# zixinz990/quaternion-mpc

Measured on AMD Instinct MI355X. Metric: MPC QP solves/sec (Go1, 12 forces, N=10), higher is better.
Workload: dtype f64

## Files before the change

quaternion-mpc_amd/csrc/qmpc_device.h:

```cpp
#pragma once

#include <hip/hip_runtime.h>
#include <stdint.h>

#include "../../include/qmpc.h"
#include "qmpc_params_dev.h"

namespace qmpc {

constexpr int kWave = 64;

template <class... Tables>
hipError_t set_max_lds(const Tables&... tables) {
  hipError_t e = hipSuccess;
  auto one = [&e](const auto& table) {
    for (auto k : table)
      if (e == hipSuccess) e = hipFuncSetAttribute(reinterpret_cast<const void*>(k), hipFuncAttributeMaxDynamicSharedMemorySize, 160 * 1024);
  };
  (one(tables), ...);
  return e;
}

constexpr int LD = 16;
constexpr int MAT = 12 * LD;
// ... 55 lines not shown
  L.total = (o + 1) & ~1;
  return L;
}

enum {
  C_FOOT = 0,
  C_GB = 12,
  C_WD0 = 15,
  C_CR = 18,
  C_CON = 36,
  C_X0 = 40,
};

#define QSYNC() __syncthreads()

__device__ __forceinline__ void mtm_load(const double* X, const double* Y, int lane, d4& acc) {
  const double x0 = X[lane], x1 = X[64 + lane], x2 = X[128 + lane];
  const double y0 = Y[lane], y1 = Y[64 + lane], y2 = Y[128 + lane];
  acc = __builtin_amdgcn_mfma_f64_16x16x4f64(x0, y0, acc, 0, 0, 0);
  acc = __builtin_amdgcn_mfma_f64_16x16x4f64(x1, y1, acc, 0, 0, 0);
  acc = __builtin_amdgcn_mfma_f64_16x16x4f64(x2, y2, acc, 0, 0, 0);
}
__device__ __forceinline__ d4 mtm3(const double X[3], const double Y[3], d4 acc) {
  acc = __builtin_amdgcn_mfma_f64_16x16x4f64(X[0], Y[0], acc, 0, 0, 0);
  acc = __builtin_amdgcn_mfma_f64_16x16x4f64(X[1], Y[1], acc, 0, 0, 0);
  acc = __builtin_amdgcn_mfma_f64_16x16x4f64(X[2], Y[2], acc, 0, 0, 0);
  return acc;
}
__device__ __forceinline__ void mtm(double* C, const double* X, const double* Y, int lane) {
  d4 acc = {0.0, 0.0, 0.0, 0.0};
  mtm_load(X, Y, lane, acc);
  C[lane] = acc[0];
  C[64 + lane] = acc[1];
  C[128 + lane] = acc[2];
}

typedef unsigned u2v __attribute__((ext_vector_type(2)));

template <int CTRL>
__device__ __forceinline__ double dpp_mov(double x) {
  if constexpr (CTRL >= 0x150 && CTRL <= 0x15F) {
    return __builtin_amdgcn_update_dpp(0.0, x, CTRL, 0xF, 0xF, true);
  } else {
    int lo = __double2loint(x), hi = __double2hiint(x);
    lo = __builtin_amdgcn_update_dpp(0, lo, CTRL, 0xF, 0xF, true);
    hi = __builtin_amdgcn_update_dpp(0, hi, CTRL, 0xF, 0xF, true);
    return __hiloint2double(hi, lo);
  }
}
__device__ __forceinline__ void swap16(double x, double& even, double& odd) {
  const u2v lo = __builtin_amdgcn_permlane16_swap((unsigned)__double2loint(x), (unsigned)__double2loint(x), false, false);
  const u2v hi = __builtin_amdgcn_permlane16_swap((unsigned)__double2hiint(x), (unsigned)__double2hiint(x), false, false);
  even = __hiloint2double((int)hi[0], (int)lo[0]);
  odd = __hiloint2double((int)hi[1], (int)lo[1]);
}
__device__ __forceinline__ void swap32(double x, double& lower, double& upper) {
  const u2v lo = __builtin_amdgcn_permlane32_swap((unsigned)__double2loint(x), (unsigned)__double2loint(x), false, false);
  const u2v hi = __builtin_amdgcn_permlane32_swap((unsigned)__double2hiint(x), (unsigned)__double2hiint(x), false, false);
  lower = __hiloint2double((int)hi[0], (int)lo[0]);
  upper = __hiloint2double((int)hi[1], (int)lo[1]);
}
template <int G>
__device__ __forceinline__ double rowgroup_bcast(double x) {
  double ev, od, lo, up;
  swap16(x, ev, od);
  swap32((G & 1) ? od : ev, lo, up);
  return (G & 2) ? up : lo;
}

struct OpMin { __device__ __forceinline__ double operator()(double a, double b) const { return fmin(a, b); } };
struct OpMax { __device__ __forceinline__ double operator()(double a, double b) const { return fmax(a, b); } };
struct OpSum { __device__ __forceinline__ double operator()(double a, double b) const { return a + b; } };
template <class Op>
__device__ __forceinline__ double wave_reduce(double v, Op op) {
  v = op(v, dpp_mov<0xB1>(v));
  v = op(v, dpp_mov<0x4E>(v));
  v = op(v, dpp_mov<0x141>(v));
  v = op(v, dpp_mov<0x140>(v));
  double a, b;
  swap16(v, a, b);
  v = op(a, b);
  swap32(v, a, b);
  return op(a, b);
}
__device__ __forceinline__ double wave_min(double v) { return wave_reduce(v, OpMin()); }
__device__ __forceinline__ double wave_max(double v) { return wave_reduce(v, OpMax()); }
__device__ __forceinline__ double wave_sum(double v) { return wave_reduce(v, OpSum()); }

__device__ __forceinline__ double fast_rcp(double x) {
  double r = __builtin_amdgcn_rcp(x);
  r = fma(fma(-x, r, 1.0), r, r);
  r = fma(fma(-x, r, 1.0), r, r);
  return r;
}

__device__ __forceinline__ double fast_rsqrt(double x) {
  double r = __builtin_amdgcn_rsq(x);
  r = r * fma(-0.5 * x * r, r, 1.5);
  r = r * fma(-0.5 * x * r, r, 1.5);
  return r;
}

template <int J>
__device__ __forceinline__ double row_bcast(double x) {
  return dpp_mov<0x150 + J>(x);
}
template <int J, int ROWS>
__device__ __forceinline__ double row_bcast_rows(double x, double keep) {
  return __builtin_amdgcn_update_dpp(keep, x, 0x150 + J, ROWS, 0xF, false);
}
__device__ __forceinline__ double read_lane(double x, int l) {
  const int lo = __builtin_amdgcn_readlane(__double2loint(x), l);
  const int hi = __builtin_amdgcn_readlane(__double2hiint(x), l);
  return __hiloint2double(hi, lo);
}

__device__ __forceinline__ void quat_G(const double* q, double G[12]) {
  const double s = q[0], x = q[1], y = q[2], z = q[3];
  G[0] = -x; G[1] = -y;  G[2] = -z;
  G[3] = s;  G[4] = -z;  G[5] = y;
  G[6] = z;  G[7] = s;   G[8] = -x;
  G[9] = -y; G[10] = x;  G[11] = s;
}
__device__ __forceinline__ void quat_Omega(const double* w, double O[16]) {
  const double x = w[0], y = w[1], z = w[2];
  O[0] = 0;  O[1] = -x; O[2] = -y;  O[3] = -z;
  O[4] = x;  O[5] = 0;  O[6] = z;   O[7] = -y;
  O[8] = y;  O[9] = -z; O[10] = 0;  O[11] = x;
  O[12] = z; O[13] = y; O[14] = -x; O[15] = 0;
}

template <int NL, bool LEAN>
struct ModelRegsT {
  double gb[3], wd0[3], rm[LEAN ? 3 * NL : 9 * NL];
  __device__ __forceinline__ void load(const double* cst, const double* bw0) {
    typedef Dim<NL> D;
#pragma unroll
    for (int i = 0; i < 3; ++i) { gb[i] = cst[D::C_GB + i]; wd0[i] = cst[D::C_WD0 + i]; }
    if (LEAN) {
#pragma unroll
      for (int i = 0; i < 3 * NL; ++i) rm[i] = cst[D::C_CON + i / 3] * cst[D::C_FOOT + i];
    } else {
#pragma unroll
      for (int i = 0; i < 9 * NL; ++i) rm[i] = bw0[i];
    }
  }
};

template <int NL, bool LEAN>
__device__ __forceinline__ void srbd_step(const DevParams& P, const ModelRegsT<NL, LEAN>& M, const double* x,
                                          const double* u, double* xn) {
  double F[3], vd[3], wd[3];
  {
    double f0[2] = {0, 0}, f1[2] = {0, 0}, f2[2] = {0, 0};
#pragma unroll
    for (int l = 0; l < NL; ++l) { f0[l & 1] += u[3 * l]; f1[l & 1] += u[3 * l + 1]; f2[l & 1] += u[3 * l + 2]; }
    F[0] = f0[0] + f0[1]; F[1] = f1[0] + f1[1]; F[2] = f2[0] + f2[1];
    if (LEAN) {
      double t0[2] = {0, 0}, t1[2] = {0, 0}, t2[2] = {0, 0};
#pragma unroll
      for (int l = 0; l < NL; ++l) {
        const double* r = &M.rm[3 * l];
        const double* f = &u[3 * l];
        t0[l & 1] += r[1] * f[2] - r[2] * f[1];
        t1[l & 1] += r[2] * f[0] - r[0] * f[2];
        t2[l & 1] += r[0] * f[1] - r[1] * f[0];
// ... 684 lines not shown
```

quaternion-mpc_amd/csrc/qmpc_wform.h:

```cpp
#pragma once

namespace qmpc {


struct LayoutW {
  int GK, WR, SLW;
};
constexpr int kGK = 27;
template <int NL = 4>
__host__ __device__ inline size_t wform_slice(int N, bool sl_global = false) {
  return ((size_t)N * (13 * 12 + 21 * NL + kGK + (sl_global ? 18 * NL : 0)) + 1 + 1) & ~(size_t)1;
}
template <int NL = 4>
__host__ __device__ inline Layout make_layout_w(int N, LayoutW* W, bool kd_global = false, bool sl_global = false, bool cv = false,
                                                bool full = false) {
  Layout L;
  int o = 0;
  auto take = [&](int n) { int r = o; o += n; return r; };
  constexpr int nu = 3 * NL, nc = 6 * NL, nl = NL;
  L.cst = take(NL == 4 ? 64 : 80);
  L.bw0 = take(3 * nu);
  L.refp = take(13);
  L.uref = take(nu);
  L.X = take((N + 1) * 13);
  L.U = take(N * nu);
  L.Xc = take((N + 1) * 13);
  L.dU = take(N * nu);
  const bool lean = ((NL == 8) && !full) || sl_global;
  if (sl_global) {
    L.S = 0; L.LAM = N * nc; L.RC = 2 * N * nc;
  } else {
    L.S = take(N * nc);
    L.LAM = take(N * nc);
  }
  L.DS = lean ? -1 : take(N * nc);
  L.DLAM = lean ? -1 : take(N * nc);
  if (!sl_global) L.RC = take(N * nc);
  L.AB = take(N * kAB);
  L.XT = take((N + 1) * kXT);
  if (kd_global) {
    L.KD = 0; L.ROT = N * 13 * 12; W->GK = N * (13 * 12 + 21 * nl);
    W->SLW = (N * (13 * 12 + 21 * nl + kGK) + 1 + 1) & ~1;
  } else {
    L.KD = take(N * 13 * 12);
    L.ROT = take(N * 21 * nl);
    W->GK = take(N * kGK + 1);
  }
  W->WR = take(N * 6);
  L.CV = cv ? take(N * 8) : -1;
  L.tile = sl_global ? L.X : L.S;
  L.total = (o + 1) & ~1;
  return L;
}
template <int NL = 4>
__device__ __forceinline__ int zeta_slot(int k, int i) { return 21 * NL * k + 21 * (i / 3) + 18 + (i % 3); }

constexpr int S6I_(int i, int j) { return i * 6 - i * (i - 1) / 2 + (j - i); }
__host__ __device__ constexpr int S6I(int i, int j) { return i <= j ? S6I_(i, j) : S6I_(j, i); }

enum { WM_QUAT = 0, WM_CONVEX = 1 };
__host__ __device__ constexpr int cvperm(int r) { return r < 3 ? r + 3 : (r < 6 ? r - 3 : (r < 9 ? r + 3 : r - 3)); }
__device__ __forceinline__ void cv_step_w(const DevParams& P, const double* x, const double w[6], double* xn) {
  double s0, c0, w00, w01, w11;
  sincos(x[2], &s0, &c0);
  ConvexModel::winv(P, c0, s0, w00, w01, w11);
  const double vd[3] = {w[0] * P.inv_mass, w[1] * P.inv_mass, w[2] * P.inv_mass - 9.81};
  const double wd0[3] = {w00 * w[3] + w01 * w[4], w01 * w[3] + w11 * w[4], P.Iinv[8] * w[5]};
  const double yawm = x[2] + P.hh * x[8];
  const double wm[3] = {x[6] + P.hh * wd0[0], x[7] + P.hh * wd0[1], x[8] + P.hh * wd0[2]};
  double sm_, cm_;
  sincos(yawm, &sm_, &cm_);
  ConvexModel::winv(P, cm_, sm_, w00, w01, w11);
  const double wdm[3] = {w00 * w[3] + w01 * w[4], w01 * w[3] + w11 * w[4], P.Iinv[8] * w[5]};
  xn[0] = x[0] + P.h * (cm_ * wm[0] + sm_ * wm[1]);
  xn[1] = x[1] + P.h * (-sm_ * wm[0] + cm_ * wm[1]);
  xn[2] = x[2] + P.h * wm[2];
#pragma unroll
  for (int a = 0; a < 3; ++a) {
    xn[3 + a] = x[3 + a] + P.h * (x[9 + a] + P.hh * vd[a]);
    xn[6 + a] = x[6 + a] + P.h * wdm[a];
    xn[9 + a] = x[9 + a] + P.h * vd[a];
  }
  xn[12] = 0.0;
}
__device__ __forceinline__ void cv_winv_mul(const double* W, const double t[3], double y[3]) {
  y[0] = W[0] * t[0] + W[1] * t[1];
  y[1] = W[1] * t[0] + W[2] * t[1];
  y[2] = W[3] * t[2];
}

template <bool AL = false, int NL = 4, int MD = WM_QUAT, bool LEAN = (NL == 8)>
__device__ inline void prepass_w(const DevParams& P, const Layout& L, double* sm, const double* sl,
                                 double* ROT, double* GK, double target, int lane, unsigned kapbits = 0) {
  typedef Dim<NL> D;
  constexpr int LSH = (NL == 8) ? 3 : 2;
  static_assert(NL == 4 || NL == 8, "contact points per knot: one lane quad or two");
  const int N = P.N;
  const double* cst = sm + L.cst;
  double cr[18];
#pragma unroll
  for (int i = 0; i < 18; ++i) cr[i] = cst[D::C_CR + i];
  for (int q0 = 0; q0 < NL * N; q0 += kWave) {
    const int q = q0 + lane;
    const bool live = q < NL * N;
    const int k = live ? (q >> LSH) : 0, l = q & (NL - 1);
    double* out = ROT + D::ROT * k + 21 * l;
    double acc[kGK];
#pragma unroll
    for (int i = 0; i < kGK; ++i) acc[i] = 0.0;
    const bool stance = live && cst[D::C_CON + l] != 0.0;
    if (live && !stance) {
      out[0] = 1; out[1] = 0; out[2] = 0; out[3] = 0; out[4] = 1; out[5] = 0; out[6] = 0; out[7] = 0; out[8] = 1;
      out[9] = 0; out[10] = 0; out[11] = 0; out[12] = 1; out[13] = 1; out[14] = 1; out[15] = 0; out[16] = 0; out[17] = 0;
    }
    if (stance) {
      const int lr = (NL == 4) ? l : (l & 3);
      const double R0 = P.R[3 * lr], R1 = P.R[3 * lr + 1], R2 = P.R[3 * lr + 2];
      double w[6], gi[6];
#pragma unroll
      for (int i = 0; i < 6; ++i) {
        const double lam = sl[L.LAM + D::NC * k + 6 * l + i];
        const double rc = sl[L.RC + D::NC * k + 6 * l + i];
        if (AL) {
          const double z = lam + target * rc;
          w[i] = (z > 0.0) ? target : 0.0;
          gi[i] = (z > 0.0) ? z : 0.0;
        } else {
          const double s = sl[L.S + D::NC * k + 6 * l + i];
          const double kap = LEAN ? (((kapbits >> (6 * (q0 >> 6) + i)) & 1u) ? 1.0 : 0.0) : sl[L.DS + D::NC * k + 6 * l + i];
          const double is = fast_rcp(s);
          w[i] = lam * is;
          gi[i] = (target + lam * rc) * is - kap * lam;
        }
      }
      int i1 = 0;
      double w1 = w[0];
#pragma unroll
      for (int i = 1; i < 6; ++i) if (w[i] > w1) { w1 = w[i]; i1 = i; }
      int i2 = -1;
      double w2 = -1.0;
#pragma unroll
      for (int i = 0; i < 6; ++i) {
        const bool skip = (i == i1) || ((i1 >= 4) && (i >= 4));
        if (!skip && w[i] > w2) { w2 = w[i]; i2 = i; }
      }
      double a1[3] = {0, 0, 0}, a2[3] = {0, 0, 0};
#pragma unroll
      for (int i = 0; i < 6; ++i)
#pragma unroll
        for (int a = 0; a < 3; ++a) {
          a1[a] = (i == i1) ? cr[3 * i + a] : a1[a];
          a2[a] = (i == i2) ? cr[3 * i + a] : a2[a];
        }
      const double in1 = fast_rsqrt(a1[0] * a1[0] + a1[1] * a1[1] + a1[2] * a1[2]);
      double q1[3], q2[3], q3[3];
#pragma unroll
      for (int a = 0; a < 3; ++a) q1[a] = a1[a] * in1;
#pragma unroll
      for (int pass = 0; pass < 2; ++pass) {
        const double dp = a2[0] * q1[0] + a2[1] * q1[1] + a2[2] * q1[2];
#pragma unroll
        for (int a = 0; a < 3; ++a) a2[a] -= dp * q1[a];
      }
      const double in2 = fast_rsqrt(a2[0] * a2[0] + a2[1] * a2[1] + a2[2] * a2[2]);
#pragma unroll
      for (int a = 0; a < 3; ++a) q2[a] = a2[a] * in2;
      q3[0] = q1[1] * q2[2] - q1[2] * q2[1];
      q3[1] = q1[2] * q2[0] - q1[0] * q2[2];
      q3[2] = q1[0] * q2[1] - q1[1] * q2[0];
      double T[9];
#pragma unroll
      for (int a = 0; a < 3; ++a) { T[3 * a] = q1[a]; T[3 * a + 1] = q2[a]; T[3 * a + 2] = q3[a]; }
      const double Rl[3] = {R0, R1, R2};
      const double* u = sm + L.U + D::NU * k + 3 * l;
      const double* ur = sm + L.uref + 3 * l;
      const double ru[3] = {R0 * (u[0] - ur[0]), R1 * (u[1] - ur[1]), R2 * (u[2] - ur[2])};
      double gq[3];
      double d00, d01, d02, d11, d12, d22;
      {
        double tr[9];
#pragma unroll
        for (int i = 0; i < 9; ++i) tr[i] = T[i] * Rl[i / 3];
        d00 = tr[0] * T[0] + tr[3] * T[3] + tr[6] * T[6];
        d01 = tr[0] * T[1] + tr[3] * T[4] + tr[6] * T[7];
        d02 = tr[0] * T[2] + tr[3] * T[5] + tr[6] * T[8];
        d11 = tr[1] * T[1] + tr[4] * T[4] + tr[7] * T[7];
        d12 = tr[1] * T[2] + tr[4] * T[5] + tr[7] * T[8];
        d22 = tr[2] * T[2] + tr[5] * T[5] + tr[8] * T[8];
      }
#pragma unroll
      for (int a = 0; a < 3; ++a) gq[a] = T[a] * ru[0] + T[3 + a] * ru[1] + T[6 + a] * ru[2];
#pragma unroll
      for (int i = 0; i < 6; ++i) {
        double at[3];
#pragma unroll
        for (int b = 0; b < 3; ++b) at[b] = T[b] * cr[3 * i] + T[3 + b] * cr[3 * i + 1] + T[6 + b] * cr[3 * i + 2];
#pragma unroll
        for (int a = 0; a < 3; ++a) gq[a] += gi[i] * at[a];
        const double w0 = w[i] * at[0], w1_ = w[i] * at[1];
        d00 += w0 * at[0]; d01 += w0 * at[1]; d02 += w0 * at[2];
        d11 += w1_ * at[1]; d12 += w1_ * at[2];
        d22 += w[i] * at[2] * at[2];
      }
      const double id0 = fast_rcp(d00);
      const double l10 = d01 * id0, l20 = d02 * id0;
      const double e11 = d11 - l10 * d01;
      const double id1 = fast_rcp(e11);
      const double e21 = d12 - l20 * d01;
      const double l21 = e21 * id1;
      const double e22 = d22 - l20 * d02 - l21 * e21;
      const double id2 = fast_rcp(e22);
#pragma unroll
      for (int i = 0; i < 9; ++i) out[i] = T[i];
      out[9] = l10; out[10] = l20; out[11] = l21; out[12] = id0; out[13] = id1; out[14] = id2;
      out[15] = gq[0]; out[16] = gq[1]; out[17] = gq[2];
      double V[18];
#pragma unroll
      for (int i = 0; i < 9; ++i) V[i] = T[i];
      {
        const double* bw = sm + L.bw0 + 3 * l;
#pragma unroll
        for (int a = 0; a < 3; ++a)
#pragma unroll
          for (int b = 0; b < 3; ++b)
            V[9 + 3 * a + b] = bw[D::NU * a] * T[b] + bw[D::NU * a + 1] * T[3 + b] + bw[D::NU * a + 2] * T[6 + b];
        if (MD == WM_CONVEX) {
          const double* Wk = sm + L.CV + 8 * k;
#pragma unroll
          for (int b = 0; b < 3; ++b) {
            const double t3[3] = {V[9 + b], V[12 + b], V[15 + b]};
            double y[3];
            cv_winv_mul(Wk, t3, y);
            V[9 + b] = y[0]; V[12 + b] = y[1]; V[15 + b] = y[2];
          }
        }
      }
      const double y0 = gq[0], y1 = gq[1] - l10 * y0, y2 = gq[2] - l20 * y0 - l21 * y1;
      const double z0 = id0 * y0, z1 = id1 * y1, z2 = id2 * y2;
      double v0[6], v1[6], v2[6];
#pragma unroll
      for (int i = 0; i < 6; ++i) {
        v0[i] = V[3 * i];
        v1[i] = V[3 * i + 1] - l10 * v0[i];
        v2[i] = V[3 * i + 2] - l20 * v0[i] - l21 * v1[i];
        acc[21 + i] = v0[i] * z0 + v1[i] * z1 + v2[i] * z2;
      }
#pragma unroll
      for (int i = 0; i < 6; ++i) {
        const double b0 = id0 * v0[i], b1 = id1 * v1[i], b2 = id2 * v2[i];
#pragma unroll
        for (int j = i; j < 6; ++j) acc[S6I(i, j)] = b0 * v0[j] + b1 * v1[j] + b2 * v2[j];
      }
    }
#pragma unroll
    for (int i = 0; i < kGK; ++i) {
      double v = acc[i];
      v += dpp_mov<0xB1>(v);
      v += dpp_mov<0x4E>(v);
      if (NL == 8) v += dpp_mov<0x141>(v);
      acc[i] = v;
    }
    if (live && l == 0) {
      double* gk = GK + kGK * k;
#pragma unroll
      for (int i = 0; i < kGK; ++i) gk[i] = acc[i];
    }
  }
  QSYNC();
}

template <bool PROF>
__device__ __forceinline__ void tick_dep(Prof<PROF>& prof, int ph, double& a, double& b) {
  if (PROF) {
    asm volatile("s_nop 0" : "+v"(a), "+v"(b));
    prof.tick(ph);
    asm volatile("s_nop 0" : "+v"(a), "+v"(b));
  }
}

template <bool PROF>
__device__ __forceinline__ void tick_dep1(Prof<PROF>& prof, int ph, double& a) {
  if (PROF) {
    asm volatile("s_nop 0" : "+v"(a));
    prof.tick(ph);
    asm volatile("s_nop 0" : "+v"(a));
  }
}

__device__ __forceinline__ d4 mtm2(const double X[2], const double Y[2], d4 acc) {
  acc = __builtin_amdgcn_mfma_f64_16x16x4f64(X[0], Y[0], acc, 0, 0, 0);
  acc = __builtin_amdgcn_mfma_f64_16x16x4f64(X[1], Y[1], acc, 0, 0, 0);
  return acc;
}
__device__ __forceinline__ d4 acc_rows(double a, double b) {
  d4 v;
  v[0] = a; v[1] = b;
  return v;
}
__device__ __forceinline__ d4 acc_rows(double a, double b, double c) {
  d4 v;
  v[0] = a; v[1] = b; v[2] = c;
  return v;
}
struct ColOps {
  double m1c, m2c, keep, hsel;
  __device__ __forceinline__ void init(const DevParams& P, int c) {
    const double m1 = P.h * (P.hh * (1.0 / P.mass)), m2 = P.h * (1.0 / P.mass);
    m1c = (c < 3) ? m1 : 0.0;
    m2c = (c < 3) ? m2 : ((c < 6) ? P.h : 0.0);
    keep = (c >= 3 && c < 6) ? 0.0 : 1.0;
    hsel = (c >= 6 && c < 9) ? P.h : 0.0;
  }
};
constexpr int kZeroSlots = 54;
template <int NL> __host__ __device__ constexpr int kZeroSlotsT() { return NL == 4 ? kZeroSlots : 70; }
struct BwPat {
  ColOps co;
  double Mc[3], Nc[2], qadd[3], sel[3];
  int ix_w, st_w, ix_a, st_a, ix_x[3], st_x[3], ix_g[2], st_g[2], kwo[2], xoffN[3];
  bool c12;
  template <int NL = 4, int MD = WM_QUAT>
  __device__ __forceinline__ void init(const DevParams& P, const Layout& L, int lane) {
    const int N = P.N;
    const int c = lane & 15, g = lane >> 4;
    co.init(P, c);
    const int zs = L.cst + kZeroSlotsT<NL>();
    const bool c35 = (c >= 3 && c < 6), c911 = (c >= 9 && c < 12);
    c12 = c == 12;
    const int abN = L.AB + kAB * (N - 1);
    ix_w = c35 ? abN + 18 + (c - 3) : zs;   st_w = c35 ? kAB : 0;
    ix_a = c35 ? abN + (c - 3) : (c911 ? abN + 9 + (c - 9) : zs);   st_a = (c35 || c911) ? kAB : 0;
    sel[0] = (g == 3) ? 1.0 : 0.0;
    sel[1] = (g == 0) ? 1.0 : 0.0;
    sel[2] = (g == 1) ? 1.0 : 0.0;
    const double m1 = P.h * (P.hh * (1.0 / P.mass)), m2 = P.h * (1.0 / P.mass);
#pragma unroll
    for (int e = 0; e < 3; ++e) {
      const int r = 4 * e + g;
      const bool phi = (r >= 3 && r < 6);
      double v = 0.0;
      if (c < 6) {
        if (r < 3) v = (r == c) ? m1 : 0.0;
        else if (r >= 6 && r < 9) v = (r - 6 == c) ? m2 : 0.0;
        else if (r >= 9) v = (r - 9 == c - 3) ? P.h : 0.0;
      }
      Mc[e] = v;
      if (MD == WM_CONVEX) qadd[e] = (c < 12 && r == c) ? P.Q[cvperm(r < 12 ? r : 0)] : 0.0;
      else qadd[e] = (c < 12 && r == c && !phi) ? P.Q[(r < 3) ? r : r + 1] : 0.0;
      const bool xv = (MD == WM_CONVEX) ? c12 : ((phi && c35) || c12);
      const int xo = c12 ? 9 + r : 3 * (r - 3) + (c - 3);
      xoffN[e] = xv ? xo : -1;
      ix_x[e] = xv ? L.XT + kXT * (N - 1) + xo : zs;
      st_x[e] = xv ? kXT : 0;
    }
#pragma unroll
    for (int e = 0; e < 2; ++e) {
      const int r = 4 * e + g;
      const bool phi = (r >= 3 && r < 6);
      Nc[e] = (r < 3 && c == r + 6) ? P.h : ((phi && r == c) ? -1.0 : 0.0);
      const bool gv = r < 6 && (c < 6 || c12);
      const int go = c12 ? 21 + r : S6I(r < 6 ? r : 0, c < 6 ? c : 0);
      ix_g[e] = gv ? kGK * (N - 1) + go : kGK * N;
      st_g[e] = gv ? kGK : 0;
      kwo[e] = (r < 6 && c < 13) ? 13 * r + c : -1;
    }
  }
};
__device__ __forceinline__ void fma_bcast345_x2(double r[2], const double x[2], const double sh[2], double cs, const double m[3]) {
  asm("v_fmac_f64 %0, %4, %5\n\t"
      "v_fmac_f64 %1, %4, %6\n\t"
      "v_fmac_f64_dpp %0, %2, %7 row_newbcast:3 row_mask:0xf bank_mask:0xf\n\t"
      "v_fmac_f64_dpp %1, %3, %7 row_newbcast:3 row_mask:0xf bank_mask:0xf\n\t"
      "v_fmac_f64_dpp %0, %2, %8 row_newbcast:4 row_mask:0xf bank_mask:0xf\n\t"
      "v_fmac_f64_dpp %1, %3, %8 row_newbcast:4 row_mask:0xf bank_mask:0xf\n\t"
      "v_fmac_f64_dpp %0, %2, %9 row_newbcast:5 row_mask:0xf bank_mask:0xf\n\t"
      "v_fmac_f64_dpp %1, %3, %9 row_newbcast:5 row_mask:0xf bank_mask:0xf"
      : "+v"(r[0]), "+v"(r[1])
      : "v"(x[0]), "v"(x[1]), "v"(cs), "v"(sh[0]), "v"(sh[1]), "v"(m[0]), "v"(m[1]), "v"(m[2]));
}
__device__ __forceinline__ void fma_bcast345_x3(double r[3], const double x[3], const double sh[3], double cs, const double m[3]) {
  asm("v_fmac_f64 %0, %6, %7\n\t"
      "v_fmac_f64 %1, %6, %8\n\t"
      "v_fmac_f64 %2, %6, %9\n\t"
      "v_fmac_f64_dpp %0, %3, %10 row_newbcast:3 row_mask:0xf bank_mask:0xf\n\t"
      "v_fmac_f64_dpp %1, %4, %10 row_newbcast:3 row_mask:0xf bank_mask:0xf\n\t"
      "v_fmac_f64_dpp %2, %5, %10 row_newbcast:3 row_mask:0xf bank_mask:0xf\n\t"
      "v_fmac_f64_dpp %0, %3, %11 row_newbcast:4 row_mask:0xf bank_mask:0xf\n\t"
      "v_fmac_f64_dpp %1, %4, %11 row_newbcast:4 row_mask:0xf bank_mask:0xf\n\t"
      "v_fmac_f64_dpp %2, %5, %11 row_newbcast:4 row_mask:0xf bank_mask:0xf\n\t"
      "v_fmac_f64_dpp %0, %3, %12 row_newbcast:5 row_mask:0xf bank_mask:0xf\n\t"
      "v_fmac_f64_dpp %1, %4, %12 row_newbcast:5 row_mask:0xf bank_mask:0xf\n\t"
      "v_fmac_f64_dpp %2, %5, %12 row_newbcast:5 row_mask:0xf bank_mask:0xf"
      : "+v"(r[0]), "+v"(r[1]), "+v"(r[2])
      : "v"(x[0]), "v"(x[1]), "v"(x[2]), "v"(cs), "v"(sh[0]), "v"(sh[1]), "v"(sh[2]), "v"(m[0]), "v"(m[1]), "v"(m[2]));
}
__device__ __forceinline__ void times_M(const double x[2], const ColOps& co, const double wt[3], double r[2]) {
  double sh[2];
#pragma unroll
// ... 644 lines not shown
    o[0] = du[0]; o[1] = du[1]; o[2] = du[2];
    bad = bad || !(isfinite(du[0]) && isfinite(du[1]) && isfinite(du[2]));
    stp = fmax(stp, fmax(fabs(du[0]), fmax(fabs(du[1]), fabs(du[2]))));
#pragma unroll
    for (int i = 0; i < 6; ++i) {
      const double jd = cr[3 * i] * du[0] + cr[3 * i + 1] * du[1] + cr[3 * i + 2] * du[2];
      double dsv = -(jd + rc[i]);
      double dlv = (target - (1.0 + kap[i]) * sv[i] * lv[i] - lv[i] * dsv) * fast_rcp(sv[i]);
      dsv = stance ? dsv : 0.0;
      dlv = stance ? dlv : 0.0;
      const bool up = (dsv < 0.0) && (pd == 0.0 || sv[i] * pd < pn * (-dsv));
      pn = up ? sv[i] : pn; pd = up ? -dsv : pd;
      const bool ud = (dlv < 0.0) && (dd == 0.0 || lv[i] * dd < dn * (-dlv));
      dn = ud ? lv[i] : dn; dd = ud ? -dlv : dd;
      if (!LEAN) {
        sl[L.DS + i0 + i] = dsv;
        sl[L.DLAM + i0 + i] = dlv;
      }
      bits |= (stance && kap[i] != 0.0) ? (1u << (6 * j + i)) : 0u;
    }
  }
  const double ap = (pd > 0.0) ? fmin(1.0, P.tau * pn * fast_rcp(pd)) : 1.0;
  const double ad = (dd > 0.0) ? fmin(1.0, P.tau * dn * fast_rcp(dd)) : 1.0;
  *alpha_p = wave_min(ap);
  *alpha_d = wave_min(ad);
  *full_step = wave_max(stp);
  kapbits = bits;
  QSYNC();
  return __any(bad ? 1 : 0);
}

template <int NL = 4, bool LEAN = (NL == 8)>
__device__ inline void apply_w(const DevParams& P, const Layout& L, double* sl, double ap, double ad, unsigned conmask,
                               int lane, unsigned& kapbits, double& sl_part, double& rc_part, const double* sm = nullptr,
                               double target = 0.0) {
  typedef Dim<NL> D;
  constexpr int LSH = (NL == 8) ? 3 : 2;
  const int N = P.N;
  sl_part = 0.0;
  rc_part = 0.0;
  const bool full = (ap >= 0.99) && (ad >= 0.99);
  const double rcs = (ap >= 1.0) ? 0.0 : (1.0 - ap);
  int j = 0;
  for (int q = lane; q < NL * N; q += kWave, ++j) {
    const int k = q >> LSH, l = q & (NL - 1);
    if (!(conmask & (1u << l))) continue;
    const int i0 = D::NC * k + 6 * l;
    double s0[6], l0[6], ds[6], dl[6], rc[6];
#pragma unroll
    for (int i = 0; i < 6; ++i) {
      s0[i] = sl[L.S + i0 + i]; l0[i] = sl[L.LAM + i0 + i]; rc[i] = sl[L.RC + i0 + i];
      if (!LEAN) { ds[i] = sl[L.DS + i0 + i]; dl[i] = sl[L.DLAM + i0 + i]; }
    }
    if (LEAN) {
      const double* cr = sm + L.cst + D::C_CR;
      const double* du = sm + L.dU + D::NU * k + 3 * l;
      const double du0 = du[0], du1 = du[1], du2 = du[2];
#pragma unroll
      for (int i = 0; i < 6; ++i) {
        const double kp = ((kapbits >> (6 * j + i)) & 1u) ? 1.0 : 0.0;
        const double jd = cr[3 * i] * du0 + cr[3 * i + 1] * du1 + cr[3 * i + 2] * du2;
        ds[i] = -(jd + rc[i]);
        dl[i] = (target - (1.0 + kp) * s0[i] * l0[i] - l0[i] * ds[i]) * fast_rcp(s0[i]);
      }
    }
    unsigned newbits = 0;
#pragma unroll
    for (int i = 0; i < 6; ++i) {
      const bool kap0 = (kapbits >> (6 * j + i)) & 1u;
      const double s1 = s0[i] + ap * ds[i];
      const double l1 = l0[i] + ad * dl[i];
      const double rc1 = (ap >= 1.0) ? 0.0 : rcs * rc[i];
      sl[L.S + i0 + i] = s1;
      sl[L.RC + i0 + i] = rc1;
      sl[L.LAM + i0 + i] = l1;
      sl_part += s1 * l1;
      rc_part = fmax(rc_part, fabs(rc1));
      const bool sig = full && (s1 < 0.6 * s0[i]) && (l1 < 0.6 * l0[i]) && (kap0 || ((s1 > 0.4 * s0[i]) && (l1 > 0.4 * l0[i])));
      if (LEAN) newbits |= sig ? (1u << (6 * j + i)) : 0u;
      else sl[L.DS + i0 + i] = sig ? 1.0 : 0.0;
    }
    if (LEAN) kapbits = (kapbits & ~(63u << (6 * j))) | newbits;
  }
}

__device__ __forceinline__ int trial_states_slot(const Layout& L, int g) {
  return g == 0 ? L.Xc + 13 : (g == 1 ? L.S : (g == 2 ? L.DLAM : L.XT));
}
template <int MD = WM_QUAT, int NL = 4>
__device__ inline double rollout_trials_w(const DevParams& P, const Layout& L, const LayoutW& LW, double* sm,
                                          const double* KD, double* ZG, double alpha_g, int lane) {
  typedef typename std::conditional<MD == WM_CONVEX, ConvexModel, typename std::conditional<NL == 8, Quat8Model, QuatModel>::type>::type TM;
  typedef Dim<NL> D;
  const int N = P.N;
  const double* cst = sm + L.cst;
  double gb[3], wd0[3];
#pragma unroll
  for (int a = 0; a < 3; ++a) { gb[a] = cst[D::C_GB + a]; wd0[a] = cst[D::C_WD0 + a]; }
  const int r = lane & 15, g = lane >> 4;
  const int row = (r < 12) ? r : 0, wi = (r < 6) ? r : 0;
  double* zg = ZG + 6 * N * g;
  double* xg = sm + trial_states_slot(L, g);
  double xc[13], xn[13];
#pragma unroll
  for (int i = 0; i < 13; ++i) xc[i] = cst[D::C_X0 + i];
  if (lane == 15)
#pragma unroll
    for (int i = 0; i < 13; ++i) sm[L.Xc + i] = xc[i];
  double Jx = TM::knot_cost(P, sm + L.refp, sm + L.uref, 0, xc, nullptr);
  auto knot = [&](int k, RollLoadsW& cur) {
    roll_load_w(L, LW, sm, KD, k, row, wi, cur);
    double dx[12], e[12];
    if (MD == WM_CONVEX) {
#pragma unroll
      for (int rr = 0; rr < 12; ++rr) dx[rr] = xc[cvperm(rr)] - cur.xo[cvperm(rr)];
    } else {
      QuatModel::state_diff(cur.xo, xc, dx);
    }
#pragma unroll
    for (int a = 0; a < 3; ++a) {
      e[a] = dx[a] + P.h * dx[6 + a];
      e[3 + a] = (cur.ab[3 * a] * dx[3] + cur.ab[3 * a + 1] * dx[4] + cur.ab[3 * a + 2] * dx[5]) +
                 (cur.ab[9 + 3 * a] * dx[9] + cur.ab[9 + 3 * a + 1] * dx[10] + cur.ab[9 + 3 * a + 2] * dx[11]);
      e[6 + a] = dx[6 + a];
      e[9 + a] = dx[9 + a];
    }
    const double* kd = cur.kd;
    const double p0 = alpha_g * kd[12] + kd[0] * e[0] + kd[1] * e[1] + kd[2] * e[2];
    const double p1 = kd[3] * e[3] + kd[4] * e[4] + kd[5] * e[5];
    const double p2 = kd[6] * e[6] + kd[7] * e[7] + kd[8] * e[8];
    const double p3 = kd[9] * e[9] + kd[10] * e[10] + kd[11] * e[11];
    const double s = (p0 + p1) + (p2 + p3);
    const double wn = (MD == WM_CONVEX) ? s : cur.wk + s;
    if (r >= 6 && r < 12) zg[6 * k + r - 6] = s;
    double w[6];
    w[0] = dpp_mov<0x150>(wn); w[1] = dpp_mov<0x151>(wn); w[2] = dpp_mov<0x152>(wn);
    w[3] = dpp_mov<0x153>(wn); w[4] = dpp_mov<0x154>(wn); w[5] = dpp_mov<0x155>(wn);
    if (MD == WM_CONVEX) {
      RollLoadsC rc;
      roll_load_c(L, LW, sm, k, rc);
      const double d3 = rc.iw[0] * w[3] + rc.iw[1] * w[4], d4 = rc.iw[1] * w[3] + rc.iw[2] * w[4], d5 = rc.iw[3] * w[5];
      w[0] += rc.wr[0]; w[1] += rc.wr[1]; w[2] += rc.wr[2];
      w[3] = rc.wr[3] + d3; w[4] = rc.wr[4] + d4; w[5] = rc.wr[5] + d5;
      cv_step_w(P, xc, w, xn);
    } else
    srbd_step_w(P, gb, wd0, xc, w, xn);
#pragma unroll
    for (int i = 0; i < 13; ++i) xc[i] = xn[i];
    if (r == 15)
#pragma unroll
      for (int i = 0; i < 13; ++i) xg[13 * k + i] = xn[i];
    Jx += TM::knot_cost(P, sm + L.refp, sm + L.uref, k + 1, xc, nullptr);
  };
  RollLoadsW ra;
  for (int k = 0; k < N; ++k) knot(k, ra);
  QSYNC();
  return Jx;
}

template <int MD = WM_QUAT, int NL = 4>
__device__ inline void trial_inputs_w(const DevParams& P, const Layout& L, const double* sm, const double* sl,
                                      const double* ROT, const double* ZG, const double* Rl, double alpha, double rho,
                                      int lane, double Ju[4], double mer[4], double vi[4]) {
  typedef Dim<NL> D;
  constexpr int LSH = (NL == 8) ? 3 : 2;
  const int N = P.N;
// ... 139 lines not shown
```

quaternion-mpc_amd/csrc/qmpc_wform_body.inc:

```
#ifndef QMPC_WNL
#define QMPC_WNL 4
#define QMPC_WNL_DEFAULTED 1
#endif
#ifndef QMPC_WMODEL
#define QMPC_WMODEL WM_QUAT
#define QMPC_WMODEL_DEFAULTED 1
#endif
  constexpr int WNL = QMPC_WNL;
  constexpr int WMT = QMPC_WMODEL;
  typedef typename std::conditional<WMT == WM_CONVEX, ConvexModel, QuatModelT<WNL>>::type WMD;
  typedef Dim<WNL> WD;
  constexpr int NU = WD::NU, NC = WD::NC;
  const int N = P.N;
  constexpr bool KDG = WVAR == 5 || WVAR == 6;
  constexpr bool SLG = WVAR == 6;
  constexpr bool LEAN = WNL == 8 || SLG;
  LayoutW LW;
  const Layout L = make_layout_w<WNL>(N, &LW, KDG, SLG, WMT == WM_CONVEX);
  double* wsb = KDG ? gws + (size_t)wslot * wform_slice<WNL>(N, SLG) : sm;
  double* KD = wsb + L.KD;
  double* ROT = wsb + L.ROT;
  double* GK = wsb + LW.GK;
  double* sl = SLG ? wsb + LW.SLW : sm;
  const void* in = reinterpret_cast<const double*>(in_) + (size_t)b * WD::REC;
  int status = QMPC_OK;
  Prof<PROF> prof;
  prof.start();
  setup_instance<WMD>(P, L, sm, in, lane, &status);
  if (status != QMPC_OK) {
    if (lane < NU) forces[NU * (size_t)b + lane] = 0.0;
    if (lane == 0 && info) {
      qmpc_info r = {status, 0, 0.0, 0.0, 0.0, 0.0};
      info[b] = r;
    }
    if (traj_u) for (int i = lane; i < N * NU; i += kWave) traj_u[(size_t)b * N * NU + i] = 0.0;
    if (traj_x) for (int i = lane; i < (N + 1) * WMD::NX; i += kWave) traj_x[(size_t)b * (N + 1) * WMD::NX + i] = 0.0;
    return;
  }
  unsigned conmask = 0;
  for (int l = 0; l < WMD::NL; ++l) conmask |= (sm[L.cst + WD::C_CON + l] != 0.0) ? (1u << l) : 0u;
  conmask = __builtin_amdgcn_readfirstlane(conmask);
  if (lane < 10) sm[L.cst + kZeroSlotsT<WNL>() + lane] = 0.0;
  if (lane == 0) GK[kGK * N] = 0.0;
  BwPat bp;
  if (!KDG) bp.init<WNL, WMT>(P, L, lane);
  if (resume) {
    for (int i = lane; i < N * NU; i += kWave) sm[L.U + i] = resume[8 + i];
  } else if (warm_t > 0) {
    if (lane < NU) {
      const bool stance = (conmask >> (lane / 3)) & 1u;
      for (int k = 0; k < N; ++k) {
        const double prev = sm[L.U + ((k + 1 < N) ? k + 1 : k) * NU + lane];
        sm[L.U + k * NU + lane] = !stance ? 0.0 : (prev != 0.0 ? prev : sm[L.uref + lane]);
      }
    }
  } else {
    for (int i = lane; i < N * NU; i += kWave) sm[L.U + i] = sm[L.uref + (i % NU)];
  }
  QSYNC();
  rollout_open<WMD, false>(P, L, sm, lane);
  wrench_from_inputs<false, WNL>(P, L, LW, sm, lane);
  expansions_w<WNL, WMT>(P, L, LW, sm, lane);
  double sl_part = 0.0, rc_part = 0.0;
  unsigned kapbits = 0;
  if (resume) {
    const double rho = resume[0];
    int j = 0;
    for (int i = lane; i < N * NC; i += kWave, ++j) {
      const int row = i % NC, l = row / 6, r = row - 6 * l;
      const double* cr = sm + L.cst + WD::C_CR + 3 * r;
      const double* ur = sm + L.uref + 3 * l;
      double c0 = cr[0] * ur[0] + cr[1] * ur[1] + cr[2] * ur[2];
      if (r == 4) c0 += -P.fz_max * sm[L.cst + WD::C_CON + l];
      const double s0 = fmax(-c0, 1.0);
      const double sraw = resume[8 + N * NU + i], lam = resume[8 + N * NU + N * NC + i];
      const double sv = fabs(sraw), rc = rho * ((resume[5] != 0.0) ? resume[8 + N * NU + 2 * N * NC + i] : (c0 + s0));
      const bool flag = sraw < 0.0;
      sl[L.S + i] = sv;
      sl[L.RC + i] = rc;
      sl[L.LAM + i] = lam;
      if (!LEAN) sl[L.DS + i] = flag ? 1.0 : 0.0;
      if (conmask & (1u << l)) {
        sl_part += sv * lam;
        rc_part = fmax(rc_part, fabs(rc));
        kapbits |= flag ? (1u << j) : 0u;
      }
    }
  } else
  for (int i = lane; i < N * NC; i += kWave) {
    const double c0 = cone_value<WD>(P, L, sm, i);
    const double s0 = fmax(-c0, 1.0);
    const double lam0 = P.mu0 / s0;
    sl[L.S + i] = s0;
    sl[L.RC + i] = c0 + s0;
    sl[L.LAM + i] = lam0;
    if (!LEAN) sl[L.DS + i] = 0.0;
    if (conmask & (1u << ((i % NC) / 6))) {
      sl_part += s0 * lam0;
      rc_part = fmax(rc_part, fabs(c0 + s0));
    }
  }
  QSYNC();
  prof.tick(PH_SETUP);
  const double inv_rows = 1.0 / (double)(6 * N * __popc(conmask));
  const int it_start = resume ? (int)resume[4] + 1 : 1;
  int it = 0, iters = it_start - 1;
  double mu = 0.0, resid = 0.0, last_step = resume ? resume[3] : 1e300, last_ap = resume ? resume[1] : 0.0,
         last_ad = resume ? resume[2] : 0.0;
  status = QMPC_MAX_ITER;
  mu = wave_sum(sl_part) * inv_rows;
  resid = wave_max(rc_part);
  for (it = it_start; it <= P.iterations_max + 1; ++it) {
    if (mu <= P.mu_final && resid <= P.tol_feas && last_step <= P.tol_step) { status = QMPC_OK; break; }
    if (it > P.iterations_max) break;
    double sg = P.sigma;
    const double amin = fmin(last_ap, last_ad);
    if (it > 1 && amin >= 0.99) sg = P.sigma_fast;
    else if (it > 1 && amin < 0.2) sg = fmax(sg, 0.8);
    else if (it > 1 && amin < 0.5) sg = fmax(sg, 0.5);
    const double target = sg * mu;
    prof.tick(PH_MISC);
    prepass_w<false, WNL, WMT, LEAN>(P, L, sm, sl, ROT, GK, target, lane, kapbits);
    prof.tick(PH_PREPASS);
    if (KDG) bp.init<WNL, WMT>(P, L, lane);
    if (backward_pass_w<PROF, false, WMT>(P, L, bp, sm, KD, GK, lane, prof)) { status = QMPC_NOT_PD; break; }
    QSYNC();
    double ap, ad;
    rollout_closed_w<PROF, !KDG, WNL, WMT>(P, L, LW, sm, KD, ROT, lane, prof);
    prof.tick(PH_ROLL);
    {
      double stp_;
      if (recover_directions_w<WNL, WMT, LEAN>(P, L, sm, sl, ROT, target, lane, &ap, &ad, &stp_, kapbits)) { status = QMPC_NOT_PD; break; }
      last_step = stp_;
    }
    last_ap = ap; last_ad = ad;
    prof.tick(PH_DIRS);
    if (LEAN) apply_w<WNL, true>(P, L, sl, ap, ad, conmask, lane, kapbits, sl_part, rc_part, sm, target);
    if (ap < 1.0) rollout_scaled_w<WNL, WMT>(P, L, LW, sm, ap, lane);
    prof.tick(PH_ROLL);
    if (!LEAN) apply_w<WNL, false>(P, L, sl, ap, ad, conmask, lane, kapbits, sl_part, rc_part);
    prof.tick(PH_APPLY);
    for (int i = lane; i < N * NU; i += kWave) sm[L.U + i] += sm[L.dU + i];
    for (int i = lane; i < (N + 1) * 13; i += kWave) sm[L.X + i] = sm[L.Xc + i];
    QSYNC();
    iters = it;
    mu = wave_sum(sl_part) * inv_rows;
    resid = wave_max(rc_part);
    if ((mu <= P.mu_final && resid <= P.tol_feas && last_step <= P.tol_step) || it >= P.iterations_max) continue;
    if (!(ap < 1.0)) wrench_from_inputs<false, WNL>(P, L, LW, sm, lane);
    prof.tick(PH_MISC);
    expansions_w<WNL, WMT>(P, L, LW, sm, lane);
    prof.tick(PH_EXPAND);
  }
  if (lane < NU) forces[NU * (size_t)b + lane] = sm[L.U + lane];
  if (traj_u) for (int i = lane; i < N * NU; i += kWave) traj_u[(size_t)b * N * NU + i] = sm[L.U + i];
  if (traj_x)
    for (int i = lane; i < (N + 1) * WMD::NX; i += kWave) {
      if (WMD::NX == 13) {
        traj_x[(size_t)b * (N + 1) * WMD::NX + i] = sm[L.X + i];
      } else {
        const int k_ = i / WMD::NX, j_ = i - WMD::NX * k_;
        traj_x[(size_t)b * (N + 1) * WMD::NX + i] = sm[L.X + 13 * k_ + j_];
      }
    }
  if (info) {
    const double J = cost_plain<WMD>(P, L, sm, lane);
    double viol = 0.0;
    for (int i = lane; i < N * NC; i += kWave) {
      const int l = (i % NC) / 6;
      if (conmask & (1u << l)) viol = fmax(viol, fmax(cone_value<WD>(P, L, sm, i), 0.0));
    }
    viol = wave_max(viol);
    if (lane == 0) {
      qmpc_info r = {status, iters, J, viol, last_step, mu};
      info[b] = r;
    }
  }
  if (PROF && prof_out && lane == 0) {
    prof.tick(PH_MISC);
#pragma unroll
    for (int i = 0; i < PH_COUNT; ++i) prof_out[16 * (size_t)b + i] = prof.t[i];
    prof_out[16 * (size_t)b + 15] = iters;
  }
#ifdef QMPC_WMODEL_DEFAULTED
#undef QMPC_WMODEL
#undef QMPC_WMODEL_DEFAULTED
#endif
#ifdef QMPC_WNL_DEFAULTED
#undef QMPC_WNL
#undef QMPC_WNL_DEFAULTED
#endif
```

Baseline: 2.001 million.

## Fuse direction recovery with iterate update and batch wave reductions

For the four-point quaternion model with local workspace, a new routine computes search directions and applies the step in one pass. The last wave chunk stays in registers and kappa flags are packed into a bitmask, which cuts shared-memory round trips between recover_directions_w and apply_w. The step-length and convergence reductions are interleaved into multi-value DPP reductions. The prepass also stops rewriting swing-leg records after the first iteration and picks constraint rows by indexed loads instead of select loops. This adds a specialized code path that must stay bit-identical to the old one.

```diff
diff --git a/quaternion-mpc_amd/csrc/qmpc_device.h b/quaternion-mpc_amd/csrc/qmpc_device.h
--- a/quaternion-mpc_amd/csrc/qmpc_device.h
+++ b/quaternion-mpc_amd/csrc/qmpc_device.h
@@ -161,6 +161,28 @@
   v = op(a, b);
   swap32(v, a, b);
   return op(a, b);
+}
+template <class OpA, class OpB>
+__device__ __forceinline__ void wave_reduce2(double& a, double& b, OpA oa, OpB ob) {
+#define QMPC_RED_STEP(CTRL) { const double ta = dpp_mov<CTRL>(a), tb = dpp_mov<CTRL>(b); a = oa(a, ta); b = ob(b, tb); }
+  QMPC_RED_STEP(0xB1) QMPC_RED_STEP(0x4E) QMPC_RED_STEP(0x141) QMPC_RED_STEP(0x140)
+#undef QMPC_RED_STEP
+  double a0, a1, b0, b1;
+  swap16(a, a0, a1); swap16(b, b0, b1);
+  a = oa(a0, a1); b = ob(b0, b1);
+  swap32(a, a0, a1); swap32(b, b0, b1);
+  a = oa(a0, a1); b = ob(b0, b1);
+}
+template <class OpA, class OpB, class OpC>
+__device__ __forceinline__ void wave_reduce3(double& a, double& b, double& c, OpA oa, OpB ob, OpC oc) {
+#define QMPC_RED_STEP(CTRL) { const double ta = dpp_mov<CTRL>(a), tb = dpp_mov<CTRL>(b), tc = dpp_mov<CTRL>(c); a = oa(a, ta); b = ob(b, tb); c = oc(c, tc); }
+  QMPC_RED_STEP(0xB1) QMPC_RED_STEP(0x4E) QMPC_RED_STEP(0x141) QMPC_RED_STEP(0x140)
+#undef QMPC_RED_STEP
+  double a0, a1, b0, b1, c0, c1;
+  swap16(a, a0, a1); swap16(b, b0, b1); swap16(c, c0, c1);
+  a = oa(a0, a1); b = ob(b0, b1); c = oc(c0, c1);
+  swap32(a, a0, a1); swap32(b, b0, b1); swap32(c, c0, c1);
+  a = oa(a0, a1); b = ob(b0, b1); c = oc(c0, c1);
 }
 __device__ __forceinline__ double wave_min(double v) { return wave_reduce(v, OpMin()); }
 __device__ __forceinline__ double wave_max(double v) { return wave_reduce(v, OpMax()); }
diff --git a/quaternion-mpc_amd/csrc/qmpc_wform.h b/quaternion-mpc_amd/csrc/qmpc_wform.h
--- a/quaternion-mpc_amd/csrc/qmpc_wform.h
+++ b/quaternion-mpc_amd/csrc/qmpc_wform.h
@@ -89,9 +89,13 @@
   y[2] = W[3] * t[2];
 }
 
-template <bool AL = false, int NL = 4, int MD = WM_QUAT, bool LEAN = (NL == 8)>
+constexpr int kZeroSlots = 54;
+template <int NL> __host__ __device__ constexpr int kZeroSlotsT() { return NL == 4 ? kZeroSlots : 70; }
+
+template <bool AL = false, int NL = 4, int MD = WM_QUAT, bool LEAN = (NL == 8), bool ROWIDX = false>
 __device__ inline void prepass_w(const DevParams& P, const Layout& L, double* sm, const double* sl,
-                                 double* ROT, double* GK, double target, int lane, unsigned kapbits = 0) {
+                                 double* ROT, double* GK, double target, int lane, unsigned kapbits = 0,
+                                 bool swing_records = true) {
   typedef Dim<NL> D;
   constexpr int LSH = (NL == 8) ? 3 : 2;
   static_assert(NL == 4 || NL == 8, "contact points per knot: one lane quad or two");
@@ -109,7 +113,7 @@
 #pragma unroll
     for (int i = 0; i < kGK; ++i) acc[i] = 0.0;
     const bool stance = live && cst[D::C_CON + l] != 0.0;
-    if (live && !stance) {
+    if (live && !stance && swing_records) {
       out[0] = 1; out[1] = 0; out[2] = 0; out[3] = 0; out[4] = 1; out[5] = 0; out[6] = 0; out[7] = 0; out[8] = 1;
       out[9] = 0; out[10] = 0; out[11] = 0; out[12] = 1; out[13] = 1; out[14] = 1; out[15] = 0; out[16] = 0; out[17] = 0;
     }
@@ -145,13 +149,20 @@
         if (!skip && w[i] > w2) { w2 = w[i]; i2 = i; }
       }
       double a1[3] = {0, 0, 0}, a2[3] = {0, 0, 0};
-#pragma unroll
-      for (int i = 0; i < 6; ++i)
-#pragma unroll
-        for (int a = 0; a < 3; ++a) {
-          a1[a] = (i == i1) ? cr[3 * i + a] : a1[a];
-          a2[a] = (i == i2) ? cr[3 * i + a] : a2[a];
-        }
+      if (ROWIDX) {
+        const double* r1 = cst + D::C_CR + 3 * i1;
+        const double* r2 = cst + ((i2 >= 0) ? D::C_CR + 3 * i2 : kZeroSlotsT<NL>());
+#pragma unroll
+        for (int a = 0; a < 3; ++a) { a1[a] = r1[a]; a2[a] = r2[a]; }
+      } else {
+#pragma unroll
+        for (int i = 0; i < 6; ++i)
+#pragma unroll
+          for (int a = 0; a < 3; ++a) {
+            a1[a] = (i == i1) ? cr[3 * i + a] : a1[a];
+            a2[a] = (i == i2) ? cr[3 * i + a] : a2[a];
+          }
+      }
       const double in1 = fast_rsqrt(a1[0] * a1[0] + a1[1] * a1[1] + a1[2] * a1[2]);
       double q1[3], q2[3], q3[3];
 #pragma unroll
@@ -312,8 +323,6 @@
     hsel = (c >= 6 && c < 9) ? P.h : 0.0;
   }
 };
-constexpr int kZeroSlots = 54;
-template <int NL> __host__ __device__ constexpr int kZeroSlotsT() { return NL == 4 ? kZeroSlots : 70; }
 struct BwPat {
   ColOps co;
   double Mc[3], Nc[2], qadd[3], sel[3];
@@ -1124,6 +1133,145 @@
     }
     if (LEAN) kapbits = (kapbits & ~(63u << (6 * j))) | newbits;
   }
+}
+
+template <int NL = 4, int MD = WM_QUAT>
+__device__ inline int directions_apply_w(const DevParams& P, const Layout& L, double* sm, double* sl, const double* ROT,
+                                         double target, unsigned conmask, int lane, double* alpha_p, double* alpha_d,
+                                         double* full_step, double& sl_part, double& rc_part) {
+  static_assert(NL == 4 && MD == WM_QUAT, "directions_apply_w: bit-identical to recover_directions_w + apply_w for QuatMpc's four points only");
+  typedef Dim<NL> D;
+  constexpr int LSH = 2;
+  const int N = P.N;
+  const int NQ = NL * N, q_last = ((NQ - 1) >> 6) << 6;
+  const double* cr = sm + L.cst + D::C_CR;
+  const bool on = (conmask >> (lane & (NL - 1))) & 1u;
+  bool bad = false;
+  double pn = 1.0, pd = 0.0, dn = 1.0, ddn = 0.0;
+  double stp = 0.0;
+  unsigned bits = 0;
+  double sv[6], lv[6], rc[6], nds[6], dlv[6], kap[6];
+  int j = 0;
+  for (int q0 = 0; q0 <= q_last; q0 += kWave, ++j) {
+    const int q = q0 + lane;
+    const bool last = q0 == q_last;
+    const int k = q >> LSH, l = q & (NL - 1);
+    double du[3] = {0.0, 0.0, 0.0};
+    if (on & (q < NQ)) {
+      const double* rec = ROT + D::ROT * k + 21 * l;
+      const int i0 = D::NC * k + 6 * l;
+      double T[9], z[6];
+#pragma unroll
+      for (int i = 0; i < 9; ++i) T[i] = rec[i];
+#pragma unroll
+      for (int i = 0; i < 6; ++i) z[i] = ROT[zeta_slot<NL>(k, i)];
+      const double l10 = rec[9], l20 = rec[10], l21 = rec[11], id0 = rec[12], id1 = rec[13], id2 = rec[14];
+      const double g0 = rec[15], g1 = rec[16], g2 = rec[17];
+#pragma unroll
+      for (int i = 0; i < 6; ++i) {
+        sv[i] = sl[L.S + i0 + i]; lv[i] = sl[L.LAM + i0 + i]; rc[i] = sl[L.RC + i0 + i]; kap[i] = sl[L.DS + i0 + i];
+      }
+      const double* bw = sm + L.bw0 + 3 * l;
+      double f[3];
+#pragma unroll
+      for (int b = 0; b < 3; ++b) f[b] = z[b] + (bw[b] * z[3] + bw[D::NU + b] * z[4] + bw[2 * D::NU + b] * z[5]);
+      const double t0 = g0 + (T[0] * f[0] + T[3] * f[1] + T[6] * f[2]);
+      const double t1 = g1 + (T[1] * f[0] + T[4] * f[1] + T[7] * f[2]);
+      const double t2 = g2 + (T[2] * f[0] + T[5] * f[1] + T[8] * f[2]);
+      const double y0 = t0, y1 = t1 - l10 * y0, y2 = t2 - l20 * y0 - l21 * y1;
+      const double x2 = id2 * y2;
+      const double x1 = id1 * y1 - l21 * x2;
+      const double x0 = id0 * y0 - l10 * x1 - l20 * x2;
+#pragma unroll
+      for (int a = 0; a < 3; ++a) du[a] = -(T[3 * a] * x0 + T[3 * a + 1] * x1 + T[3 * a + 2] * x2);
+      bad = bad | !(isfinite(du[0]) & isfinite(du[1]) & isfinite(du[2]));
+      stp = fmax(stp, fmax(fabs(du[0]), fmax(fabs(du[1]), fabs(du[2]))));
+#pragma unroll
+      for (int i = 0; i < 6; ++i) {
+        const double jd = fma(cr[3 * i + 2], du[2], fma(cr[3 * i], du[0], cr[3 * i + 1] * du[1]));
+        nds[i] = jd + rc[i];
+        const double dsv = -nds[i];
+        dlv[i] = (target - (1.0 + kap[i]) * sv[i] * lv[i] - lv[i] * dsv) * fast_rcp(sv[i]);
+        const bool up = (dsv < 0.0) & ((pd == 0.0) | (sv[i] * pd < pn * (-dsv)));
+        pn = up ? sv[i] : pn; pd = up ? nds[i] : pd;
+        const bool ud = (dlv[i] < 0.0) & ((ddn == 0.0) | (lv[i] * (-ddn) < dn * (-dlv[i])));
+        dn = ud ? lv[i] : dn; ddn = ud ? dlv[i] : ddn;
+      }
+      if (!last) {
+#pragma unroll
+        for (int i = 0; i < 6; ++i) {
+          sl[L.DS + i0 + i] = -nds[i];
+          sl[L.DLAM + i0 + i] = dlv[i];
+          bits |= (kap[i] != 0.0) ? (1u << (6 * j + i)) : 0u;
+        }
+      }
+    }
+    if (q < NQ) {
+      double* o = sm + L.dU + D::NU * k + 3 * l;
+      o[0] = du[0]; o[1] = du[1]; o[2] = du[2];
+    }
+  }
+  const double dd = -ddn;
+  double ap = (pd > 0.0) ? fmin(1.0, P.tau * pn * fast_rcp(pd)) : 1.0;
+  double ad = (dd > 0.0) ? fmin(1.0, P.tau * dn * fast_rcp(dd)) : 1.0;
+  wave_reduce3(ap, ad, stp, OpMin(), OpMin(), OpMax());
+  *alpha_p = ap;
+  *alpha_d = ad;
+  *full_step = stp;
+  QSYNC();
+  if (__any(bad ? 1 : 0)) return 1;
+  sl_part = 0.0;
+  rc_part = 0.0;
+  const bool full = (ap >= 0.99) & (ad >= 0.99);
+  const bool whole = __any((ap >= 1.0) ? 1 : 0);
+  const double rcs = 1.0 - ap;
+  auto rows = [&](int i0, const double* s0, const double* l0, const double* r0, const double* nd, const double* dl, const bool* kap0) {
+#pragma unroll
+    for (int i = 0; i < 6; ++i) {
+      const double s1 = fma(ap, -nd[i], s0[i]);
+      const double l1 = fma(ad, dl[i], l0[i]);
+      sl[L.S + i0 + i] = s1;
+      sl[L.LAM + i0 + i] = l1;
+      sl_part = fma(s1, l1, sl_part);
+      const bool sig = full & (s1 < 0.6 * s0[i]) & (l1 < 0.6 * l0[i]) & (kap0[i] | ((s1 > 0.4 * s0[i]) & (l1 > 0.4 * l0[i])));
+      sl[L.DS + i0 + i] = sig ? 1.0 : 0.0;
+    }
+    if (whole) {
+#pragma unroll
+      for (int i = 0; i < 6; ++i) sl[L.RC + i0 + i] = 0.0;
+    } else {
+#pragma unroll
+      for (int i = 0; i < 6; ++i) {
+        const double rc1 = rcs * r0[i];
+        sl[L.RC + i0 + i] = rc1;
+        rc_part = fmax(rc_part, fabs(rc1));
+      }
+    }
+  };
+  j = 0;
+  for (int q0 = 0; q0 < q_last; q0 += kWave, ++j) {
+    if (on) {
+      const int q = q0 + lane;
+      const int i0 = D::NC * (q >> LSH) + 6 * (q & (NL - 1));
+      double s0[6], l0[6], r0[6], nd[6], dl[6];
+      bool kp[6];
+#pragma unroll
+      for (int i = 0; i < 6; ++i) {
+        s0[i] = sl[L.S + i0 + i]; l0[i] = sl[L.LAM + i0 + i]; r0[i] = sl[L.RC + i0 + i];
+        nd[i] = -sl[L.DS + i0 + i]; dl[i] = sl[L.DLAM + i0 + i];
+        kp[i] = (bits >> (6 * j + i)) & 1u;
+      }
+      rows(i0, s0, l0, r0, nd, dl, kp);
+    }
+  }
+  if (on & (q_last + lane < NQ)) {
+    const int q = q_last + lane;
+    bool kp[6];
+#pragma unroll
+    for (int i = 0; i < 6; ++i) kp[i] = kap[i] != 0.0;
+    rows(D::NC * (q >> LSH) + 6 * (q & (NL - 1)), sv, lv, rc, nds, dlv, kp);
+  }
+  return 0;
 }
 
 __device__ __forceinline__ int trial_states_slot(const Layout& L, int g) {
diff --git a/quaternion-mpc_amd/csrc/qmpc_wform_body.inc b/quaternion-mpc_amd/csrc/qmpc_wform_body.inc
--- a/quaternion-mpc_amd/csrc/qmpc_wform_body.inc
+++ b/quaternion-mpc_amd/csrc/qmpc_wform_body.inc
@@ -15,6 +15,7 @@
   constexpr bool KDG = WVAR == 5 || WVAR == 6;
   constexpr bool SLG = WVAR == 6;
   constexpr bool LEAN = WNL == 8 || SLG;
+  constexpr bool FUSED = !LEAN && !KDG && WMT == WM_QUAT;
   LayoutW LW;
   const Layout L = make_layout_w<WNL>(N, &LW, KDG, SLG, WMT == WM_CONVEX);
   double* wsb = KDG ? gws + (size_t)wslot * wform_slice<WNL>(N, SLG) : sm;
@@ -120,7 +121,7 @@
     else if (it > 1 && amin < 0.5) sg = fmax(sg, 0.5);
     const double target = sg * mu;
     prof.tick(PH_MISC);
-    prepass_w<false, WNL, WMT, LEAN>(P, L, sm, sl, ROT, GK, target, lane, kapbits);
+    prepass_w<false, WNL, WMT, LEAN, FUSED>(P, L, sm, sl, ROT, GK, target, lane, kapbits, !FUSED || it == it_start);
     prof.tick(PH_PREPASS);
     if (KDG) bp.init<WNL, WMT>(P, L, lane);
     if (backward_pass_w<PROF, false, WMT>(P, L, bp, sm, KD, GK, lane, prof)) { status = QMPC_NOT_PD; break; }
@@ -128,24 +129,40 @@
     double ap, ad;
     rollout_closed_w<PROF, !KDG, WNL, WMT>(P, L, LW, sm, KD, ROT, lane, prof);
     prof.tick(PH_ROLL);
-    {
+    if constexpr (FUSED) {
       double stp_;
-      if (recover_directions_w<WNL, WMT, LEAN>(P, L, sm, sl, ROT, target, lane, &ap, &ad, &stp_, kapbits)) { status = QMPC_NOT_PD; break; }
+      if (directions_apply_w<WNL, WMT>(P, L, sm, sl, ROT, target, conmask, lane, &ap, &ad, &stp_, sl_part, rc_part)) { status = QMPC_NOT_PD; break; }
       last_step = stp_;
-    }
-    last_ap = ap; last_ad = ad;
-    prof.tick(PH_DIRS);
-    if (LEAN) apply_w<WNL, true>(P, L, sl, ap, ad, conmask, lane, kapbits, sl_part, rc_part, sm, target);
-    if (ap < 1.0) rollout_scaled_w<WNL, WMT>(P, L, LW, sm, ap, lane);
-    prof.tick(PH_ROLL);
-    if (!LEAN) apply_w<WNL, false>(P, L, sl, ap, ad, conmask, lane, kapbits, sl_part, rc_part);
-    prof.tick(PH_APPLY);
+      last_ap = ap; last_ad = ad;
+      prof.tick(PH_DIRS);
+      if (ap < 1.0) rollout_scaled_w<WNL, WMT>(P, L, LW, sm, ap, lane);
+      prof.tick(PH_ROLL);
+    } else {
+      {
+        double stp_;
+        if (recover_directions_w<WNL, WMT, LEAN>(P, L, sm, sl, ROT, target, lane, &ap, &ad, &stp_, kapbits)) { status = QMPC_NOT_PD; break; }
+        last_step = stp_;
+      }
+      last_ap = ap; last_ad = ad;
+      prof.tick(PH_DIRS);
+      if (LEAN) apply_w<WNL, true>(P, L, sl, ap, ad, conmask, lane, kapbits, sl_part, rc_part, sm, target);
+      if (ap < 1.0) rollout_scaled_w<WNL, WMT>(P, L, LW, sm, ap, lane);
+      prof.tick(PH_ROLL);
+      if (!LEAN) apply_w<WNL, false>(P, L, sl, ap, ad, conmask, lane, kapbits, sl_part, rc_part);
+      prof.tick(PH_APPLY);
+    }
     for (int i = lane; i < N * NU; i += kWave) sm[L.U + i] += sm[L.dU + i];
     for (int i = lane; i < (N + 1) * 13; i += kWave) sm[L.X + i] = sm[L.Xc + i];
     QSYNC();
     iters = it;
-    mu = wave_sum(sl_part) * inv_rows;
-    resid = wave_max(rc_part);
+    if constexpr (FUSED) {
+      mu = sl_part; resid = rc_part;
+      wave_reduce2(mu, resid, OpSum(), OpMax());
+      mu *= inv_rows;
+    } else {
+      mu = wave_sum(sl_part) * inv_rows;
+      resid = wave_max(rc_part);
+    }
     if ((mu <= P.mu_final && resid <= P.tol_feas && last_step <= P.tol_step) || it >= P.iterations_max) continue;
     if (!(ap < 1.0)) wrench_from_inputs<false, WNL>(P, L, LW, sm, lane);
     prof.tick(PH_MISC);
```

After: 2.058 million, median of 6. 2.9% higher.
